# Ulixes-8/UNet-Implementations

Hardware: NVIDIA B200
Metric: our_unet_512_train_images_per_sec (higher is better)
Workload: dtype bf16

## Files before the change

### unet-implementations_b200/csrc/conv_common.cuh

```cuda
#pragma once
#include "common.cuh"

namespace b200 {

#ifdef B200UNET_INSTRUMENT
constexpr bool kInstr = true;
#else
constexpr bool kInstr = false;
#endif
constexpr int kProducerWarps = 4;
constexpr int kMmaWarp = 4;
constexpr int kEpiWarp0 = 5;
constexpr int kConvThreads = 32 * (kEpiWarp0 + 4);

static inline int make_act_map(CUtensorMap* m, const __nv_bfloat16* base, int64_t pitch, int N, int H, int W, int C,
                        int hstep, int wstep, int hoff, int woff, int boxC, int boxW, int boxH) {
  const int Hs = (H - hoff + hstep - 1) / hstep;
  const int Ws = (W - woff + wstep - 1) / wstep;
  if (Hs <= 0 || Ws <= 0) return set_error(kErrInvalid, "empty sub-lattice");
  uint64_t dims[4] = {(uint64_t)C, (uint64_t)Ws, (uint64_t)Hs, (uint64_t)N};
  uint64_t strides[3] = {(uint64_t)(wstep * pitch * 2), (uint64_t)(hstep * (int64_t)W * pitch * 2),
                         (uint64_t)((int64_t)H * W * pitch * 2)};
  uint32_t box[4] = {(uint32_t)boxC, (uint32_t)boxW, (uint32_t)boxH, 1};
  const CUtensorMapSwizzle swz = (boxC * 2 == 128) ? CU_TENSOR_MAP_SWIZZLE_128B
                                 : (boxC * 2 == 64) ? CU_TENSOR_MAP_SWIZZLE_64B
                                                    : CU_TENSOR_MAP_SWIZZLE_NONE;
  if (swz == CU_TENSOR_MAP_SWIZZLE_NONE) return set_error(kErrInvalid, "box channel count %d unsupported", boxC);
  return make_tmap_bf16(m, base + ((int64_t)hoff * W + woff) * pitch, 4, dims, strides, box, swz);
}

static inline int make_weight_map(CUtensorMap* m, const void* w, int rows, int K, int boxK, int boxRows) {
  uint64_t dims[2] = {(uint64_t)K, (uint64_t)rows};
  uint64_t strides[1] = {(uint64_t)K * 2};
  uint32_t box[2] = {(uint32_t)boxK, (uint32_t)boxRows};
  return make_tmap_bf16(m, w, 2, dims, strides, box,
                        boxK == 64 ? CU_TENSOR_MAP_SWIZZLE_128B : CU_TENSOR_MAP_SWIZZLE_64B);
}

static inline int pick_bn(int n_total) {
  if (n_total % 256 == 0) return 256;
  if (n_total % 128 == 0) return 128;
  if (n_total % 64 == 0) return 64;
  if (n_total % 32 == 0) return 32;
  return 0;
}
static inline int pick_bn_gconv(int n_total, int bk) {
  if (n_total == 96 && bk == 32) return 96;
  if ((n_total == 192 || n_total == 384) && bk == 64) return 192;
  return pick_bn(n_total);
}
static inline int pick_bk(int c) { return c % 64 == 0 ? 64 : (c % 32 == 0 ? 32 : 0); }


int launch_wgrad_finalize(const float* partial, float* dw, int S, int cin, int cout, cudaStream_t st);

struct BwdSums {
  const __nv_bfloat16* y;
  int64_t y_pitch;
  const float* a;
  const float* b;
  float slope;
};

bool nconv_supported(int k_channels, int n_channels, int stride, int W);
int nconv_stat_slots(int N, int H, int W);
int nconv_launch(const void* src, int64_t src_pitch, const void* wpack, void* out, int64_t out_pitch, float* stats, int N,
                 int H, int W, int k_channels, int n_channels, int rev, int stat_slots, cudaStream_t st,
                 const BwdSums* bs = nullptr);
bool pconv_supported(int k_channels, int n_channels, int stride, int W, int64_t src_pitch, int64_t out_pitch);
int pconv_stat_slots(int N, int H, int W);
int pconv_launch(const void* src, const void* wpack, void* out, float* stats, int N, int H, int W, int rev, int stat_slots,
                 cudaStream_t st, const BwdSums* bs = nullptr);
int conv_stat_slots(int N, int OH, int OW, int Cout);

bool wgradn_supported(int Cin, int Cout, int stride);
int64_t wgradn_workspace_bytes(int N, int H, int W, int Cin, int Cout);
int wgradn_launch(const b200unet_conv_wgrad_args* a, cudaStream_t st);

}
```

### unet-implementations_b200/csrc/conv_fprop_dgrad.cu

```cuda
#include "common.cuh"
#include "ptx.cuh"
#include "conv_common.cuh"
#include <stdlib.h>

namespace b200 {

constexpr int kTH = 16, kTW = 8;
constexpr int kMaxLoads = 4;
constexpr int kMaxTaps = 9;

struct ALoad {
  int dh, dw;
  int rows, cols;
  int ntaps;
  uint32_t a_hi;
  uint32_t mt_step16;
  uint32_t winoff16[kMaxTaps];
  int koff[kMaxTaps];
};

struct GConvParams {
  int N, OH, OW, tiles_w, tiles_h;
  int nloads, ntaps_total;
  int s1;
// ... 691 lines not shown
  GC(32, 256, 4, 4, false)
  GC(32, 128, 8, 4, false)
  GC(32, 96, 8, 4, false)
  GC(32, 96, 8, 1, true)
  GC(32, 64, 8, 4, false)
  GC(32, 64, 8, 1, true)
  GC(32, 32, 8, 4, false)
  GC(32, 32, 8, 1, true)
#undef GC
  return set_error(kErrUnsupported, "no gconv instantiation for BK=%d BN=%d", BK, BN);
}

}

using namespace b200;

extern "C" int b200unet_conv_fprop_partials(int N, int OH, int OW, int Cout) { return conv_stat_slots(N, OH, OW, Cout); }

extern "C" int b200unet_conv_fprop(const b200unet_conv_fprop_args* a, void* stream) {
  B200_CHECK_ARG(a && a->x && a->w && a->y, "conv_fprop: null pointer");
  B200_CHECK_ARG(a->stride == 1 || a->stride == 2, "conv_fprop: stride %d unsupported", a->stride);
  const int BK = pick_bk(a->Cin), BN = pick_bn_gconv(a->Cout, BK);
  if (!BK || !BN)
    return set_error(kErrUnsupported, "conv_fprop: Cin=%d Cout=%d outside the tensor-core envelope (multiples of 32)",
                     a->Cin, a->Cout);
  B200_CHECK_ARG(a->x_pitch % 8 == 0 && a->y_pitch % 8 == 0, "conv_fprop: pitches must be multiples of 8 elements");
  if (nconv_supported(a->Cin, a->Cout, a->stride, a->W))
    return nconv_launch(a->x, a->x_pitch, a->w, a->y, a->y_pitch, a->stats, a->N, a->H, a->W, a->Cin, a->Cout, 0,
                        conv_stat_slots(a->N, a->H, a->W, a->Cout), static_cast<cudaStream_t>(stream));
  const int s = a->stride;
  const int OH = (a->H - 1) / s + 1, OW = (a->W - 1) / s + 1;
  GConvParams p{};
  GConvMaps maps;
  p.N = a->N;
  p.OH = OH;
  p.OW = OW;
  p.mt = pick_mt(BK, BN, a->Cout, a->Cin, 9);
  p.tiles_w = ceil_div(OW, kTW);
  p.tiles_h = ceil_div(OH, kTH * p.mt);
  p.cin = a->Cin;
  p.cout = a->Cout;
  p.stats = a->stats;
  const __nv_bfloat16* x = static_cast<const __nv_bfloat16*>(a->x);
  TapSpec taps[9];
  SrcLattice lat[4];
  int rc;
  if (s == 1) {
    lat[0] = SrcLattice{x, a->x_pitch, a->N, a->H, a->W, a->Cin, 1, 1, 0, 0};
    int n = 0;
    for (int kw = 0; kw < 3; ++kw)
      for (int kh = 0; kh < 3; ++kh) taps[n++] = TapSpec{0, kh - 1, kw - 1, (kh * 3 + kw) * a->Cin};
  } else {
    B200_CHECK_ARG(a->H >= 2 && a->W >= 2, "conv_fprop: stride-2 input must be at least 2x2");
    for (int hp = 0; hp < 2; ++hp)
      for (int wp = 0; wp < 2; ++wp)
        lat[hp * 2 + wp] = SrcLattice{x, a->x_pitch, a->N, a->H, a->W, a->Cin, 2, 2, hp, wp};
    const int par[3] = {1, 0, 1}, sh[3] = {-1, 0, 0};
    int n = 0;
    for (int kw = 0; kw < 3; ++kw)
      for (int kh = 0; kh < 3; ++kh)
        taps[n++] = TapSpec{par[kh] * 2 + par[kw], sh[kh], sh[kw], (kh * 3 + kw) * a->Cin};
  }
  if ((rc = build_loads(taps, 9, lat, BK, &p, &maps))) return rc;
  const WSpec ws{a->w, a->Cout, 9 * a->Cin};
  const int OC = (BN % 64 == 0) ? 64 : 32;
  if ((rc = make_act_map(&maps.out[0], static_cast<const __nv_bfloat16*>(a->y), a->y_pitch, a->N, OH, OW, a->Cout, 1, 1, 0,
                         0, OC, kTW, kTH)))
    return rc;
  return dispatch_gconv(maps, p, ws, BK, BN, static_cast<cudaStream_t>(stream));
}

extern "C" int b200unet_conv_dgrad_bwd_slots(int N, int H, int W, int Cin, int Cout, int stride) {
  if (N <= 0 || H <= 0 || W <= 0) return 0;
  return nconv_supported(Cout, Cin, stride, W) ? nconv_stat_slots(N, H, W) : 0;
}

extern "C" int b200unet_conv_dgrad(const b200unet_conv_dgrad_args* a, void* stream) {
  B200_CHECK_ARG(a && a->dy && a->wt && a->dx, "conv_dgrad: null pointer");
  B200_CHECK_ARG(a->stride == 1 || a->stride == 2, "conv_dgrad: stride %d unsupported", a->stride);
  const int BK = pick_bk(a->Cout), BN = pick_bn_gconv(a->Cin, BK);
  if (!BK || !BN)
    return set_error(kErrUnsupported, "conv_dgrad: Cin=%d Cout=%d outside the tensor-core envelope", a->Cin, a->Cout);
  B200_CHECK_ARG(a->dx_pitch % 8 == 0 && a->dy_pitch % 8 == 0, "conv_dgrad: pitches must be multiples of 8 elements");
  if (nconv_supported(a->Cout, a->Cin, a->stride, a->W) && !a->dx2) {
    if (a->bs_part) {
      B200_CHECK_ARG(a->bs_y && a->bs_a && a->bs_b, "conv_dgrad: norm-backward sums need y, a and b");
      BwdSums bs{static_cast<const __nv_bfloat16*>(a->bs_y), a->bs_y_pitch, a->bs_a, a->bs_b, a->bs_slope};
      return nconv_launch(a->dy, a->dy_pitch, a->wt, a->dx, a->dx_pitch, a->bs_part, a->N, a->H, a->W, a->Cout, a->Cin, 1,
                          nconv_stat_slots(a->N, a->H, a->W), static_cast<cudaStream_t>(stream), &bs);
    }
    return nconv_launch(a->dy, a->dy_pitch, a->wt, a->dx, a->dx_pitch, nullptr, a->N, a->H, a->W, a->Cout, a->Cin, 1, 0,
                        static_cast<cudaStream_t>(stream));
  }
  B200_CHECK_ARG(!a->bs_part, "conv_dgrad: this shape does not produce norm-backward sums (b200unet_conv_dgrad_bwd_slots == 0)");
  const int s = a->stride;
  const int OH = (a->H - 1) / s + 1, OW = (a->W - 1) / s + 1;
  const __nv_bfloat16* dy = static_cast<const __nv_bfloat16*>(a->dy);
  const __nv_bfloat16* dx = static_cast<const __nv_bfloat16*>(a->dx);
  const int OC = (BN % 64 == 0) ? 64 : 32;
  cudaStream_t st = static_cast<cudaStream_t>(stream);
  int rc;
  GConvMaps maps;
  const WSpec ws{a->wt, a->Cin, 9 * a->Cout};
  SrcLattice lat[1] = {SrcLattice{dy, a->dy_pitch, a->N, OH, OW, a->Cout, 1, 1, 0, 0}};
  if (s == 1) {
    GConvParams p{};
    p.N = a->N;
    p.OH = a->H;
    p.OW = a->W;
    p.mt = pick_mt(BK, BN, a->Cin, a->Cout, 9);
    p.tiles_w = ceil_div(a->W, kTW);
    p.tiles_h = ceil_div(a->H, kTH * p.mt);
    p.cin = a->Cout;
    p.cout = a->Cin;
    p.stats = nullptr;
    TapSpec taps[9];
    int n = 0;
    for (int kw = 0; kw < 3; ++kw)
      for (int kh = 2; kh >= 0; --kh) taps[n++] = TapSpec{0, 1 - kh, 1 - kw, (kh * 3 + kw) * a->Cout};
    if ((rc = build_loads(taps, 9, lat, BK, &p, &maps))) return rc;
    if (a->dx2) {
      B200_CHECK_ARG(a->dx_split > 0 && a->dx_split < a->Cin && a->dx_split % OC == 0 && a->Cin / OC <= 8 && BN == a->Cin,
                     "conv_dgrad: dx_split=%d must be a multiple of %d inside (0, %d), one N tile", a->dx_split, OC, a->Cin);
      B200_CHECK_ARG(a->dx2_pitch % 8 == 0, "conv_dgrad: dx2 pitch must be a multiple of 8 elements");
      p.out_split = OC;
      const __nv_bfloat16* dx2 = static_cast<const __nv_bfloat16*>(a->dx2);
      for (int j = 0; j < a->Cin / OC; ++j) {
        const int c0 = j * OC;
        const bool first = c0 < a->dx_split;
        if ((rc = make_act_map(&maps.out[j], first ? dx + c0 : dx2 + (c0 - a->dx_split), first ? a->dx_pitch : a->dx2_pitch,
                               a->N, a->H, a->W, OC, 1, 1, 0, 0, OC, kTW, kTH)))
          return rc;
      }
      return dispatch_gconv(maps, p, ws, BK, BN, st);
    }
    if ((rc = make_act_map(&maps.out[0], dx, a->dx_pitch, a->N, a->H, a->W, a->Cin, 1, 1, 0, 0, OC, kTW, kTH))) return rc;
    return dispatch_gconv(maps, p, ws, BK, BN, st);
  }
  B200_CHECK_ARG(!a->dx2, "conv_dgrad: a split output needs stride 1");
  for (int ph = 0; ph < 2; ++ph)
    for (int pw = 0; pw < 2; ++pw) {
      const int Hs = (a->H - ph + 1) / 2, Ws = (a->W - pw + 1) / 2;
      if (Hs <= 0 || Ws <= 0) continue;
      GConvParams p{};
      p.N = a->N;
      p.OH = Hs;
      p.OW = Ws;
      p.mt = pick_mt(BK, BN, a->Cin, a->Cout, (ph ? 2 : 1) * (pw ? 2 : 1));
      p.tiles_w = ceil_div(Ws, kTW);
      p.tiles_h = ceil_div(Hs, kTH * p.mt);
      p.cin = a->Cout;
      p.cout = a->Cin;
      p.stats = nullptr;
      int khs[2], dhs[2], nkh, kws[2], dws[2], nkw;
      if (ph == 0) { nkh = 1; khs[0] = 1; dhs[0] = 0; } else { nkh = 2; khs[0] = 0; dhs[0] = 1; khs[1] = 2; dhs[1] = 0; }
      if (pw == 0) { nkw = 1; kws[0] = 1; dws[0] = 0; } else { nkw = 2; kws[0] = 0; dws[0] = 1; kws[1] = 2; dws[1] = 0; }
      TapSpec taps[4];
      int n = 0;
      for (int j = 0; j < nkw; ++j)
        for (int i = 0; i < nkh; ++i) taps[n++] = TapSpec{0, dhs[i], dws[j], (khs[i] * 3 + kws[j]) * a->Cout};
      if ((rc = build_loads(taps, n, lat, BK, &p, &maps))) return rc;
      if ((rc = make_act_map(&maps.out[0], dx, a->dx_pitch, a->N, a->H, a->W, a->Cin, 2, 2, ph, pw, OC, kTW, kTH)))
        return rc;
      if ((rc = dispatch_gconv(maps, p, ws, BK, BN, st))) return rc;
    }
  return 0;
// ... 71 lines not shown
```

### unet-implementations_b200/csrc/conv_narrow.cu

```cuda
#include "common.cuh"
#include "ptx.cuh"
#include "conv_common.cuh"
#include <stdlib.h>

namespace b200 {

constexpr int kNcTH = 4, kNcTW = 32, kNcValidW = 30;
constexpr int kNcPatchRows = kNcTH + 2;
constexpr int kNcProducers = 2, kNcMmaWarp = 2, kNcEpiWarp0 = 4;
constexpr int kNcMaxGroups = 3;

struct NConvParams {
  int N, H, W, tiles_w, tiles_h;
  int cin;
    int tiles_per_cta;
  int stat_slots;
  float* stats;
  long long* debug;
  BwdSums bs;
};

struct NConvMaps {
  CUtensorMap src;
  CUtensorMap w;
// ... 342 lines not shown
    tmem_dealloc(tmem_base, Cfg::kTmemCols);
  }
}

struct NConvGrid {
  int grid, tiles_per_cta, stat_slots, tiles_w, tiles_h;
};

static NConvGrid nconv_grid(int N, int H, int W) {
  NConvGrid g;
  g.tiles_w = ceil_div(W, kNcValidW);
  g.tiles_h = ceil_div(H, kNcTH);
  const long long per_img = static_cast<long long>(g.tiles_w) * g.tiles_h;
  const long long total = per_img * N;
  g.tiles_per_cta = static_cast<int>(ceil_div64(total, num_sms()));
  if (g.tiles_per_cta < 1) g.tiles_per_cta = 1;
  g.grid = static_cast<int>(ceil_div64(total, g.tiles_per_cta));
  g.stat_slots = 4 * kNcMaxGroups * (static_cast<int>(ceil_div64(per_img, g.tiles_per_cta)) + 1);
  return g;
}

static int nconv_bk(int k_channels) { return k_channels > 32 ? 64 : 32; }

bool nconv_supported(int k_channels, int n_channels, int stride, int W) {
  if (stride != 1 || (n_channels != 32 && n_channels != 64) || k_channels % 32 != 0 || k_channels <= 0) return false;
  if (W < 64) return false;
  {
    const char* e = getenv("B200UNET_NO_NCONV");
    if (e && atoi(e) == n_channels) return false;
  }
  const int BK = nconv_bk(k_channels);
  return static_cast<long long>(ceil_div(k_channels, BK)) * 3 * (3 * n_channels * BK * 2) <= 80 * 1024;
}

int nconv_stat_slots(int N, int H, int W) {
  const int a = nconv_grid(N, H, W).stat_slots, b = pconv_stat_slots(N, H, W);
  return a > b ? a : b;
}

static long long* nconv_debug_buffer() {
  static long long* buf = nullptr;
  static int state = -1;
  if (state < 0) {
    const char* e = getenv("B200UNET_GCONV_DEBUG");
    state = (e && e[0] == '1') ? 1 : 0;
    if (state) cudaMalloc(&buf, 148 * 8 * sizeof(long long));
  }
  return state ? buf : nullptr;
}

template <int BK, int CO, int A_SLOTS, bool REV, int NG>
static int launch_nconv(const NConvMaps& maps, NConvParams& p, const NConvGrid& g, cudaStream_t st) {
  using Cfg = NConvCfg<BK, CO, A_SLOTS, NG>;
  auto kern = nconv_kernel<BK, CO, A_SLOTS, REV, NG>;
  static bool attr_set = false;
  if (!attr_set) {
    B200_CUDA(cudaFuncSetAttribute(kern, cudaFuncAttributeMaxDynamicSharedMemorySize, Cfg::kSmemBytes));
    attr_set = true;
  }
  if (p.stats)
    B200_CUDA(cudaMemsetAsync(p.stats, 0, static_cast<size_t>(p.N) * p.stat_slots * CO * 2 * sizeof(float), st));
  p.debug = nconv_debug_buffer();
  if (kInstr && p.debug) cudaMemsetAsync(p.debug, 0, 148 * 8 * sizeof(long long), st);
  launch_k(kern, dim3(g.grid), dim3(Cfg::kThreads), Cfg::kSmemBytes, st, maps, p);
  B200_LAUNCH_CHECK("nconv_kernel");
  if (kInstr && p.debug) {
    long long h[8];
    cudaStreamSynchronize(st);
    cudaMemcpy(h, p.debug, sizeof(h), cudaMemcpyDeviceToHost);
    const long long tiles = g.tiles_per_cta, gt = (tiles + NG - 1) / NG;
    fprintf(stderr,
            "nconv<%d,%d,%d,%d,%d> K %d tiles/CTA %lld | per tile: producer0 wait %lld issue %lld | mma total %lld "
            "wait_tmem_empty %lld wait_a_full %lld | epilogue group 0 per ITS tile: total %lld wait_tmem_full %lld store+bar %lld\n",
            BK, CO, A_SLOTS, (int)REV, NG, p.cin, tiles, h[0] / tiles, h[1] / tiles, h[4] / tiles, h[2] / tiles, h[3] / tiles,
            h[6] / gt, h[5] / gt, h[7] / gt);
  }
  return 0;
}

int nconv_launch(const void* src, int64_t src_pitch, const void* wpack, void* out, int64_t out_pitch, float* stats, int N,
                 int H, int W, int k_channels, int n_channels, int rev, int stat_slots, cudaStream_t st, const BwdSums* bs) {
  if (pconv_supported(k_channels, n_channels, 1, W, src_pitch, out_pitch) && (!bs || bs->y_pitch == n_channels))
    return pconv_launch(src, wpack, out, stats, N, H, W, rev, stat_slots, st, bs);
  const int BK = nconv_bk(k_channels);
  const NConvGrid g = nconv_grid(N, H, W);
  NConvParams p{};
  NConvMaps maps;
  p.N = N;
  p.H = H;
  p.W = W;
  p.tiles_w = g.tiles_w;
  p.tiles_h = g.tiles_h;
  p.cin = k_channels;
  p.tiles_per_cta = g.tiles_per_cta;
  p.stat_slots = stat_slots > g.stat_slots ? stat_slots : g.stat_slots;
  p.stats = stats;
  if (bs) {
    if (!rev || !stats || bs->y_pitch % 2 != 0)
      return set_error(kErrInvalid, "nconv: the norm-backward sums need the data gradient and a partial buffer");
    p.bs = *bs;
  }
  int rc;
  if ((rc = make_act_map(&maps.src, static_cast<const __nv_bfloat16*>(src), src_pitch, N, H, W, k_channels, 1, 1, 0, 0, BK,
                         kNcTW, kNcPatchRows)))
    return rc;
  if ((rc = make_act_map(&maps.out, static_cast<const __nv_bfloat16*>(out), out_pitch, N, H, W, n_channels, 1, 1, 0, 0,
                         n_channels, kNcValidW, kNcTH)))
    return rc;
  {
    const uint64_t kc = static_cast<uint64_t>(k_channels);
    uint64_t dims[4] = {kc, 3, 3, static_cast<uint64_t>(n_channels)};
    uint64_t strides[3] = {kc * 2, 3 * kc * 2, 9 * kc * 2};
    uint32_t box[4] = {static_cast<uint32_t>(BK), 3, 1, static_cast<uint32_t>(n_channels)};
    if ((rc = make_tmap_bf16(&maps.w, wpack, 4, dims, strides, box,
                             BK == 64 ? CU_TENSOR_MAP_SWIZZLE_128B : CU_TENSOR_MAP_SWIZZLE_64B)))
      return rc;
  }
#define NC(bk, co, as, ng) \
  if (BK == bk && n_channels == co) \
    return rev ? launch_nconv<bk, co, as, true, ng>(maps, p, g, st) : launch_nconv<bk, co, as, false, ng>(maps, p, g, st);
  NC(64, 64, 4, 2) NC(64, 32, 4, 2) NC(32, 64, 8, 2) NC(32, 32, 8, 2)
#undef NC
  return set_error(kErrUnsupported, "no nconv instantiation for BK=%d N=%d", BK, n_channels);
}

}
```

### unet-implementations_b200/csrc/conv_pair.cu

```cuda
#include "common.cuh"
#include "ptx.cuh"
#include "conv_common.cuh"
#include <stdlib.h>

namespace b200 {

constexpr int kPcTH = 4, kPcTW = 32, kPcValidW = 30;
constexpr int kPcPatchRows = kPcTH + 2;
constexpr int kPcProducers = 2, kPcMmaWarp = 2, kPcEpiWarp0 = 4;
constexpr int kPcNG = 2;
constexpr int kPcStatWarp0 = kPcEpiWarp0 + 4 * kPcNG;
constexpr int kPcC = 32;
constexpr int kPcSlots = 6;

struct PConvParams {
  int N, H, Wp, tiles_w, tiles_h;
  int tiles_per_cta;
  int stat_slots;
  float* stats;
  const __nv_bfloat16* w;
  BwdSums bs;
};

struct PConvMaps {
// ... 317 lines not shown
      th = th_n;
      tw = tw_n;
      n_img = img_n;
    };
    for (int it = 0; it < n_tiles; it += 2) {
      one_tile(it, ya, yb);
      if (it + 1 < n_tiles) one_tile(it + 1, yb, ya);
    }
    if (acc_img >= 0) flush(acc_img);
  }

  tc_fence_before();
  __syncthreads();
  if (warp == kPcMmaWarp) {
    tc_fence_after();
    tmem_dealloc(tmem_base, Cfg::kTmemCols);
  }
}

struct PConvGrid {
  int grid, tiles_per_cta, stat_slots, tiles_w, tiles_h;
};

static PConvGrid pconv_grid(int N, int H, int W) {
  PConvGrid g;
  g.tiles_w = ceil_div(W / 2, kPcValidW);
  g.tiles_h = ceil_div(H, kPcTH);
  const long long per_img = static_cast<long long>(g.tiles_w) * g.tiles_h;
  const long long total = per_img * N;
  g.tiles_per_cta = static_cast<int>(ceil_div64(total, num_sms()));
  if (g.tiles_per_cta < 1) g.tiles_per_cta = 1;
  g.grid = static_cast<int>(ceil_div64(total, g.tiles_per_cta));
  g.stat_slots = 4 * kPcNG * (static_cast<int>(ceil_div64(per_img, g.tiles_per_cta)) + 1);
  return g;
}

bool pconv_supported(int k_channels, int n_channels, int stride, int W, int64_t src_pitch, int64_t out_pitch) {
  static const bool off = [] { const char* e = getenv("B200UNET_NO_PCONV"); return e && e[0] == '1'; }();
  return !off && stride == 1 && k_channels == kPcC && n_channels == kPcC && W % 2 == 0 && W >= 128 &&
         src_pitch == kPcC && out_pitch == kPcC;
}

int pconv_stat_slots(int N, int H, int W) { return (W % 2 == 0 && W >= 128) ? pconv_grid(N, H, W).stat_slots : 0; }

int pconv_launch(const void* src, const void* wpack, void* out, float* stats, int N, int H, int W, int rev, int stat_slots,
                 cudaStream_t st, const BwdSums* bs) {
  const PConvGrid g = pconv_grid(N, H, W);
  PConvParams p{};
  PConvMaps maps;
  p.N = N;
  p.H = H;
  p.Wp = W / 2;
  p.tiles_w = g.tiles_w;
  p.tiles_h = g.tiles_h;
  p.tiles_per_cta = g.tiles_per_cta;
  p.stat_slots = stat_slots > g.stat_slots ? stat_slots : g.stat_slots;
  p.stats = stats;
  p.w = static_cast<const __nv_bfloat16*>(wpack);
  if (bs) {
    if (!rev || !stats || bs->y_pitch != kPcC)
      return set_error(kErrInvalid, "pconv: the norm-backward sums need the data gradient, a partial buffer and a dense y");
    p.bs = *bs;
  }
  int rc;
  if ((rc = make_act_map(&maps.src, static_cast<const __nv_bfloat16*>(src), 64, N, H, W / 2, 64, 1, 1, 0, 0, 64, kPcTW,
                         kPcPatchRows)))
    return rc;
  if ((rc = make_act_map(&maps.out, static_cast<const __nv_bfloat16*>(out), 64, N, H, W / 2, 64, 1, 1, 0, 0, 64, kPcValidW,
                         kPcTH)))
    return rc;
  auto kern = rev ? pconv_kernel<true> : pconv_kernel<false>;
  static bool attr_set[2] = {false, false};
  if (!attr_set[rev ? 1 : 0]) {
    B200_CUDA(cudaFuncSetAttribute(kern, cudaFuncAttributeMaxDynamicSharedMemorySize, PConvCfg::kSmemBytes));
    attr_set[rev ? 1 : 0] = true;
  }
  if (p.stats)
    B200_CUDA(cudaMemsetAsync(p.stats, 0, static_cast<size_t>(p.N) * p.stat_slots * kPcC * 2 * sizeof(float), st));
  launch_k(kern, dim3(g.grid), dim3(PConvCfg::kThreads), PConvCfg::kSmemBytes, st, maps, p);
  B200_LAUNCH_CHECK("pconv_kernel");
  return 0;
}

}
```

### unet-implementations_b200/csrc/ptx.cuh

```cuda
#pragma once
#include <cuda.h>
#include <cuda_runtime.h>
#include <cuda_bf16.h>
#include <stdint.h>

namespace b200 {

__device__ __forceinline__ uint32_t smem_u32(const void* p) {
  return static_cast<uint32_t>(__cvta_generic_to_shared(p));
}

__device__ __forceinline__ bool elect_one() {
  uint32_t pred;
  asm volatile(
      "{\n\t.reg .pred P;\n\t"
      "elect.sync _|P, 0xffffffff;\n\t"
      "selp.b32 %0, 1, 0, P;\n\t}"
      : "=r"(pred));
  return pred != 0;
}

__device__ __forceinline__ void pdl_launch_dependents() { asm volatile("griddepcontrol.launch_dependents;" ::: "memory"); }
__device__ __forceinline__ void pdl_wait() { asm volatile("griddepcontrol.wait;" ::: "memory"); }

// ... 79 lines not shown
__device__ __forceinline__ void tma_store_4d(const CUtensorMap* m, const void* src, int c0, int c1, int c2, int c3) {
  asm volatile("cp.async.bulk.tensor.4d.global.shared::cta.tile.bulk_group [%0, {%2, %3, %4, %5}], [%1];" ::"l"(m),
               "r"(smem_u32(src)), "r"(c0), "r"(c1), "r"(c2), "r"(c3)
               : "memory");
}
__device__ __forceinline__ void tma_store_commit() { asm volatile("cp.async.bulk.commit_group;" ::: "memory"); }
__device__ __forceinline__ void tma_store_wait_all() { asm volatile("cp.async.bulk.wait_group 0;" ::: "memory"); }
__device__ __forceinline__ void tma_store_wait_read_all() {
  asm volatile("cp.async.bulk.wait_group.read 0;" ::: "memory");
}
__device__ __forceinline__ void tma_store_wait_read_1() {
  asm volatile("cp.async.bulk.wait_group.read 1;" ::: "memory");
}
__device__ __forceinline__ void fence_proxy_async_smem() {
  asm volatile("fence.proxy.async.shared::cta;" ::: "memory");
}

__device__ __forceinline__ void tmem_alloc(uint32_t* dst_smem, uint32_t ncols) {
  asm volatile("tcgen05.alloc.cta_group::1.sync.aligned.shared::cta.b32 [%0], %1;" ::"r"(smem_u32(dst_smem)),
               "r"(ncols)
               : "memory");
}
__device__ __forceinline__ void tmem_relinquish() {
  asm volatile("tcgen05.relinquish_alloc_permit.cta_group::1.sync.aligned;" ::: "memory");
}
__device__ __forceinline__ void tmem_dealloc(uint32_t taddr, uint32_t ncols) {
  asm volatile("tcgen05.dealloc.cta_group::1.sync.aligned.b32 %0, %1;" ::"r"(taddr), "r"(ncols) : "memory");
}
__device__ __forceinline__ void tc_fence_before() {
  asm volatile("tcgen05.fence::before_thread_sync;" ::: "memory");
}
__device__ __forceinline__ void tc_fence_after() { asm volatile("tcgen05.fence::after_thread_sync;" ::: "memory"); }

__device__ __forceinline__ void umma_bf16(uint32_t tmem_d, uint64_t adesc, uint64_t bdesc, uint32_t idesc,
                                          uint32_t accumulate) {
  asm volatile(
      "{\n\t.reg .pred p;\n\t"
      "setp.ne.b32 p, %4, 0;\n\t"
      "tcgen05.mma.cta_group::1.kind::f16 [%0], %1, %2, %3, p;\n\t}" ::"r"(tmem_d),
      "l"(adesc), "l"(bdesc), "r"(idesc), "r"(accumulate)
      : "memory");
}
__device__ __forceinline__ uint32_t umma_desc_lo(uint32_t saddr, uint32_t lbo_bytes) {
  return ((saddr >> 4) & 0x3FFFu) | (((lbo_bytes >> 4) & 0x3FFFu) << 16);
}
__host__ __device__ constexpr uint32_t umma_desc_hi(uint32_t sbo_bytes, uint32_t layout) {
  return ((sbo_bytes >> 4) & 0x3FFFu) | (1u << 14) | ((layout & 7u) << 29);
}
__device__ __forceinline__ void umma_bf16_lean(uint32_t tmem_d, uint32_t a_lo, uint32_t a_hi, uint32_t b_lo,
                                               uint32_t b_hi, uint32_t idesc, uint32_t accumulate) {
  asm volatile(
      "{\n\t.reg .pred p;\n\t.reg .b64 da, db;\n\t"
      "setp.ne.b32 p, %6, 0;\n\t"
      "mov.b64 da, {%1, %2};\n\t"
      "mov.b64 db, {%3, %4};\n\t"
      "tcgen05.mma.cta_group::1.kind::f16 [%0], da, db, %5, p;\n\t}" ::"r"(tmem_d),
      "r"(a_lo), "r"(a_hi), "r"(b_lo), "r"(b_hi), "r"(idesc), "r"(accumulate)
      : "memory");
}
__device__ __forceinline__ void umma_commit(uint64_t* bar) {
  asm volatile("tcgen05.commit.cta_group::1.mbarrier::arrive::one.shared::cluster.b64 [%0];" ::"r"(smem_u32(bar))
               : "memory");
}
__device__ __forceinline__ void tmem_ld_32x32(uint32_t taddr, uint32_t (&v)[32]) {
  asm volatile(
      "tcgen05.ld.sync.aligned.32x32b.x32.b32 "
      "{%0, %1, %2, %3, %4, %5, %6, %7, %8, %9, %10, %11, %12, %13, %14, %15, "
      "%16, %17, %18, %19, %20, %21, %22, %23, %24, %25, %26, %27, %28, %29, %30, %31}, [%32];"
      : "=r"(v[0]), "=r"(v[1]), "=r"(v[2]), "=r"(v[3]), "=r"(v[4]), "=r"(v[5]), "=r"(v[6]), "=r"(v[7]), "=r"(v[8]),
        "=r"(v[9]), "=r"(v[10]), "=r"(v[11]), "=r"(v[12]), "=r"(v[13]), "=r"(v[14]), "=r"(v[15]), "=r"(v[16]),
        "=r"(v[17]), "=r"(v[18]), "=r"(v[19]), "=r"(v[20]), "=r"(v[21]), "=r"(v[22]), "=r"(v[23]), "=r"(v[24]),
        "=r"(v[25]), "=r"(v[26]), "=r"(v[27]), "=r"(v[28]), "=r"(v[29]), "=r"(v[30]), "=r"(v[31])
      : "r"(taddr)
      : "memory");
}
__device__ __forceinline__ void tmem_ld_32x16(uint32_t taddr, uint32_t (&v)[16]) {
  asm volatile(
      "tcgen05.ld.sync.aligned.32x32b.x16.b32 "
      "{%0, %1, %2, %3, %4, %5, %6, %7, %8, %9, %10, %11, %12, %13, %14, %15}, [%16];"
      : "=r"(v[0]), "=r"(v[1]), "=r"(v[2]), "=r"(v[3]), "=r"(v[4]), "=r"(v[5]), "=r"(v[6]), "=r"(v[7]), "=r"(v[8]),
        "=r"(v[9]), "=r"(v[10]), "=r"(v[11]), "=r"(v[12]), "=r"(v[13]), "=r"(v[14]), "=r"(v[15])
      : "r"(taddr)
      : "memory");
}
__device__ __forceinline__ void tmem_ld_wait() { asm volatile("tcgen05.wait::ld.sync.aligned;" ::: "memory"); }

__device__ __forceinline__ uint32_t mapa_u32(uint32_t saddr, uint32_t rank) {
  uint32_t ra;
  asm volatile("mapa.shared::cluster.u32 %0, %1, %2;" : "=r"(ra) : "r"(saddr), "r"(rank));
  return ra;
}
__device__ __forceinline__ uint32_t cluster_ctarank() {
  uint32_t r;
  asm volatile("mov.u32 %0, %%cluster_ctarank;" : "=r"(r));
  return r;
}
__device__ __forceinline__ void cluster_sync_all() {
  asm volatile("barrier.cluster.arrive.release.aligned;" ::: "memory");
  asm volatile("barrier.cluster.wait.acquire.aligned;" ::: "memory");
}
__device__ __forceinline__ void tma_load_2d_pair(void* dst, const CUtensorMap* m, uint32_t leader_bar, int c0, int c1) {
  asm volatile(
      "cp.async.bulk.tensor.2d.cta_group::2.shared::cluster.global.mbarrier::complete_tx::bytes [%0], [%1, {%3, %4}], [%2];"
      ::"r"(smem_u32(dst)), "l"(m), "r"(leader_bar), "r"(c0), "r"(c1)
      : "memory");
}
__device__ __forceinline__ void tma_load_4d_pair(void* dst, const CUtensorMap* m, uint32_t leader_bar, int c0, int c1,
                                                 int c2, int c3) {
  asm volatile(
      "cp.async.bulk.tensor.4d.cta_group::2.shared::cluster.global.mbarrier::complete_tx::bytes [%0], [%1, {%3, %4, %5, "
      "%6}], [%2];" ::"r"(smem_u32(dst)),
      "l"(m), "r"(leader_bar), "r"(c0), "r"(c1), "r"(c2), "r"(c3)
      : "memory");
}
__device__ __forceinline__ void mbar_arrive_cluster(uint64_t* bar, uint32_t rank) {
  asm volatile(
      "{\n\t.reg .b32 ra;\n\t"
      "mapa.shared::cluster.u32 ra, %0, %1;\n\t"
      "mbarrier.arrive.release.cluster.shared::cluster.b64 _, [ra];\n\t}" ::"r"(smem_u32(bar)),
      "r"(rank)
      : "memory");
}
__device__ __forceinline__ void tmem_alloc_pair(uint32_t* dst_smem, uint32_t ncols) {
  asm volatile("tcgen05.alloc.cta_group::2.sync.aligned.shared::cta.b32 [%0], %1;" ::"r"(smem_u32(dst_smem)),
               "r"(ncols)
               : "memory");
}
__device__ __forceinline__ void tmem_relinquish_pair() {
  asm volatile("tcgen05.relinquish_alloc_permit.cta_group::2.sync.aligned;" ::: "memory");
}
__device__ __forceinline__ void tmem_dealloc_pair(uint32_t taddr, uint32_t ncols) {
  asm volatile("tcgen05.dealloc.cta_group::2.sync.aligned.b32 %0, %1;" ::"r"(taddr), "r"(ncols) : "memory");
}
__device__ __forceinline__ void umma_bf16_lean_pair(uint32_t tmem_d, uint32_t a_lo, uint32_t a_hi, uint32_t b_lo,
                                                    uint32_t b_hi, uint32_t idesc, uint32_t accumulate) {
  asm volatile(
      "{\n\t.reg .pred p;\n\t.reg .b64 da, db;\n\t"
      "setp.ne.b32 p, %6, 0;\n\t"
      "mov.b64 da, {%1, %2};\n\t"
      "mov.b64 db, {%3, %4};\n\t"
      "tcgen05.mma.cta_group::2.kind::f16 [%0], da, db, %5, p;\n\t}" ::"r"(tmem_d),
      "r"(a_lo), "r"(a_hi), "r"(b_lo), "r"(b_hi), "r"(idesc), "r"(accumulate)
      : "memory");
}
__device__ __forceinline__ void umma_commit_pair_u32(uint32_t bar) {
  asm volatile(
      "{\n\t.reg .b16 m;\n\t"
      "mov.b16 m, 3;\n\t"
      "tcgen05.commit.cta_group::2.mbarrier::arrive::one.shared::cluster.multicast::cluster.b64 [%0], m;\n\t}" ::"r"(bar)
      : "memory");
}

enum : uint32_t { kSwzNone = 0, kSwz128 = 2, kSwz64 = 4, kSwz32 = 6 };

__device__ __forceinline__ uint64_t umma_smem_desc(uint32_t saddr, uint32_t lbo_bytes, uint32_t sbo_bytes,
                                                   uint32_t layout) {
  uint64_t d = 0;
  d |= static_cast<uint64_t>((saddr >> 4) & 0x3FFF);
  d |= static_cast<uint64_t>((lbo_bytes >> 4) & 0x3FFF) << 16;
  d |= static_cast<uint64_t>((sbo_bytes >> 4) & 0x3FFF) << 32;
  d |= static_cast<uint64_t>(1) << 46;
  d |= static_cast<uint64_t>(layout & 7) << 61;
  return d;
}
__host__ __device__ constexpr uint32_t umma_idesc_bf16(int M, int N, int a_mn, int b_mn) {
  return (1u << 4) | (1u << 7) | (1u << 10) | (static_cast<uint32_t>(a_mn) << 15) |
// ... 44 lines not shown
```

Baseline: 1607.

## Add paired-column 96-channel conv kernel for fprop and dgrad

Adds a specialised tcgen05 kernel for 3x3 convolutions between 96 and 32 channels. It treats pairs of adjacent pixels as one wider pixel (W/2 lattice) so each MMA uses N=96 and the horizontal taps merge. Partial sums of neighbouring columns are combined with warp shuffles in the epilogue. Fprop fuses norm statistics in dedicated warps, and dgrad writes to split outputs through strided tensor maps. This replaces the narrow/generic paths for these shapes and adds complex swizzle and weight-repacking logic that must be correct.

```diff
diff --git a/unet-implementations_b200/csrc/conv_common.cuh b/unet-implementations_b200/csrc/conv_common.cuh
--- a/unet-implementations_b200/csrc/conv_common.cuh
+++ b/unet-implementations_b200/csrc/conv_common.cuh
@@ -71,6 +71,12 @@
 int pconv_stat_slots(int N, int H, int W);
 int pconv_launch(const void* src, const void* wpack, void* out, float* stats, int N, int H, int W, int rev, int stat_slots,
                  cudaStream_t st, const BwdSums* bs = nullptr);
+bool pconv96_fprop_supported(int k_channels, int n_channels, int stride, int W, int64_t src_pitch, int64_t out_pitch);
+int pconv96_fprop(const void* x, const void* wpack, void* y, float* stats, int N, int H, int W, int stat_slots,
+                  cudaStream_t st);
+bool pconv96_dgrad_supported(int cin, int cout, int stride, int W, int64_t dy_pitch);
+int pconv96_dgrad(const void* dy, const void* wpack, const void* const out[3], const int64_t pitch[3], int N, int H, int W,
+                  cudaStream_t st);
 int conv_stat_slots(int N, int OH, int OW, int Cout);
 
 bool wgradn_supported(int Cin, int Cout, int stride);
diff --git a/unet-implementations_b200/csrc/conv_fprop_dgrad.cu b/unet-implementations_b200/csrc/conv_fprop_dgrad.cu
--- a/unet-implementations_b200/csrc/conv_fprop_dgrad.cu
+++ b/unet-implementations_b200/csrc/conv_fprop_dgrad.cu
@@ -797,6 +797,25 @@
   if (!BK || !BN)
     return set_error(kErrUnsupported, "conv_dgrad: Cin=%d Cout=%d outside the tensor-core envelope", a->Cin, a->Cout);
   B200_CHECK_ARG(a->dx_pitch % 8 == 0 && a->dy_pitch % 8 == 0, "conv_dgrad: pitches must be multiples of 8 elements");
+  if (pconv96_dgrad_supported(a->Cin, a->Cout, a->stride, a->W, a->dy_pitch) && !a->bs_part) {
+    const __nv_bfloat16* dx = static_cast<const __nv_bfloat16*>(a->dx);
+    const void* out[3];
+    int64_t pitch[3];
+    for (int j = 0; j < 3; ++j) {
+      out[j] = dx + 32 * j;
+      pitch[j] = a->dx_pitch;
+    }
+    if (a->dx2) {
+      B200_CHECK_ARG(a->dx_split > 0 && a->dx_split < a->Cin && a->dx_split % 32 == 0,
+                     "conv_dgrad: dx_split=%d must be a multiple of 32 inside (0, %d)", a->dx_split, a->Cin);
+      B200_CHECK_ARG(a->dx2_pitch % 8 == 0, "conv_dgrad: dx2 pitch must be a multiple of 8 elements");
+      for (int j = a->dx_split / 32; j < 3; ++j) {
+        out[j] = static_cast<const __nv_bfloat16*>(a->dx2) + (32 * j - a->dx_split);
+        pitch[j] = a->dx2_pitch;
+      }
+    }
+    return pconv96_dgrad(a->dy, a->wt, out, pitch, a->N, a->H, a->W, static_cast<cudaStream_t>(stream));
+  }
   if (nconv_supported(a->Cout, a->Cin, a->stride, a->W) && !a->dx2) {
     if (a->bs_part) {
       B200_CHECK_ARG(a->bs_y && a->bs_a && a->bs_b, "conv_dgrad: norm-backward sums need y, a and b");
diff --git a/unet-implementations_b200/csrc/conv_narrow.cu b/unet-implementations_b200/csrc/conv_narrow.cu
--- a/unet-implementations_b200/csrc/conv_narrow.cu
+++ b/unet-implementations_b200/csrc/conv_narrow.cu
@@ -448,6 +448,8 @@
                  int H, int W, int k_channels, int n_channels, int rev, int stat_slots, cudaStream_t st, const BwdSums* bs) {
   if (pconv_supported(k_channels, n_channels, 1, W, src_pitch, out_pitch) && (!bs || bs->y_pitch == n_channels))
     return pconv_launch(src, wpack, out, stats, N, H, W, rev, stat_slots, st, bs);
+  if (!rev && pconv96_fprop_supported(k_channels, n_channels, 1, W, src_pitch, out_pitch))
+    return pconv96_fprop(src, wpack, out, stats, N, H, W, stat_slots, st);
   const int BK = nconv_bk(k_channels);
   const NConvGrid g = nconv_grid(N, H, W);
   NConvParams p{};
diff --git a/unet-implementations_b200/csrc/conv_pair.cu b/unet-implementations_b200/csrc/conv_pair.cu
--- a/unet-implementations_b200/csrc/conv_pair.cu
+++ b/unet-implementations_b200/csrc/conv_pair.cu
@@ -423,4 +423,435 @@
   return 0;
 }
 
-}
+constexpr int kP9K = 288;
+constexpr int kP9BTileBytes = 96 * 128;
+constexpr int kP9BTiles = kP9K / 64 + 1;
+
+template <bool REV>
+struct P9Cfg {
+  static constexpr int KC = REV ? 1 : 3;
+  static constexpr int OG = REV ? 3 : 1;
+  static constexpr int NG = REV ? 4 : 2;
+  static constexpr int kSlots = REV ? 4 : 5;
+  static constexpr int kStatWarp0 = kPcEpiWarp0 + 4 * NG;
+  static constexpr int kThreads = 32 * (kStatWarp0 + (REV ? 0 : 4));
+  static constexpr int kSlotBytes = kPcPatchRows * kPcTW * 128;
+  static constexpr int kBBytes = kP9BTiles * kP9BTileBytes;
+  static constexpr int kStageBufBytes = 16 * 1024;
+  static constexpr int kSmemBytes = kSlots * kSlotBytes + kBBytes + NG * kStageBufBytes + 1024;
+  static constexpr uint32_t kTmemCols = NG * 128;
+  static_assert(kSmemBytes <= 227 * 1024 - 256, "shared memory budget");
+};
+
+struct P9Params {
+  int N, H, Wp, tiles_w, tiles_h;
+  int tiles_per_cta;
+  int stat_slots;
+  float* stats;
+  const __nv_bfloat16* w;
+};
+
+struct P9Maps {
+  CUtensorMap src;
+  CUtensorMap out[6];
+};
+
+__device__ __forceinline__ void p9_mma(uint32_t d, uint32_t a_lo, uint32_t b_lo, bool par, bool first) {
+  constexpr uint32_t hi = umma_desc_hi(8 * 128, kSwz128);
+  constexpr uint32_t id32 = umma_idesc_bf16(128, 32, 0, 0), id64 = umma_idesc_bf16(128, 64, 0, 0),
+                     id96 = umma_idesc_bf16(128, 96, 0, 0);
+  constexpr uint32_t kRows32 = (32 * 128) >> 4, kRows64 = (64 * 128) >> 4;
+  if (!par) {
+    if (first) {
+      umma_bf16_lean(d, a_lo, hi, b_lo, hi, id32, 0u);
+      umma_bf16_lean(d + 32, a_lo, hi, b_lo + kRows32, hi, id64, 0u);
+    } else {
+      umma_bf16_lean(d, a_lo, hi, b_lo, hi, id96, 1u);
+    }
+  } else {
+    if (first) {
+      umma_bf16_lean(d + 32, a_lo, hi, b_lo, hi, id64, 1u);
+      umma_bf16_lean(d + 96, a_lo, hi, b_lo + kRows64, hi, id32, 0u);
+    } else {
+      umma_bf16_lean(d + 32, a_lo, hi, b_lo, hi, id96, 1u);
+    }
+  }
+}
+
+__device__ __forceinline__ constexpr uint32_t p9_b_off(int kk) {
+  return static_cast<uint32_t>((kk >> 6) * (kP9BTileBytes >> 4) + (((kk & 63) * 2) >> 4));
+}
+
+template <bool REV>
+__global__ void __launch_bounds__(P9Cfg<REV>::kThreads, 1) pconv96_kernel(const __grid_constant__ P9Maps maps,
+                                                                           const __grid_constant__ P9Params p) {
+  pdl_launch_dependents();
+  using Cfg = P9Cfg<REV>;
+  constexpr int KC = Cfg::KC, OG = Cfg::OG, NG = Cfg::NG, A_SLOTS = Cfg::kSlots;
+  extern __shared__ uint8_t smem_raw[];
+  __shared__ __align__(8) uint64_t a_full[A_SLOTS], a_empty[A_SLOTS];
+  __shared__ __align__(8) uint64_t b_full;
+  __shared__ __align__(8) uint64_t tmem_full_bar[NG], tmem_empty_bar[NG];
+  __shared__ uint32_t tmem_base_holder;
+
+  const int warp = threadIdx.x >> 5;
+  const int lane = threadIdx.x & 31;
+  uint8_t* smem = reinterpret_cast<uint8_t*>((reinterpret_cast<uintptr_t>(smem_raw) + 1023) & ~uintptr_t(1023));
+  uint8_t* smem_b = smem + A_SLOTS * Cfg::kSlotBytes;
+  uint8_t* staging = smem_b + Cfg::kBBytes;
+
+  const int tiles_per_img = p.tiles_w * p.tiles_h;
+  const int total_tiles = tiles_per_img * p.N;
+  const int tile_lo = min(static_cast<int>(blockIdx.x) * p.tiles_per_cta, total_tiles);
+  const int tile_hi = min(tile_lo + p.tiles_per_cta, total_tiles);
+
+  if (threadIdx.x == 0) {
+    for (int s = 0; s < A_SLOTS; ++s) {
+      mbar_init(&a_full[s], 1);
+      mbar_init(&a_empty[s], 1);
+    }
+    mbar_init(&b_full, NG * 128);
+    for (int b = 0; b < NG; ++b) {
+      mbar_init(&tmem_full_bar[b], 1);
+      mbar_init(&tmem_empty_bar[b], 4);
+    }
+    fence_barrier_init();
+  }
+  if (warp == kPcMmaWarp) {
+    tmem_alloc(&tmem_base_holder, Cfg::kTmemCols);
+    tmem_relinquish();
+  }
+  tc_fence_before();
+  __syncthreads();
+  tc_fence_after();
+  const uint32_t tmem_base = tmem_base_holder;
+  pdl_wait();
+
+  if (warp < kPcProducers) {
+    if (elect_one()) {
+      tma_prefetch_desc(&maps.src);
+      int b = 0;
+      for (int tile = tile_lo; tile < tile_hi; ++tile) {
+        const int n_img = tile / tiles_per_img;
+        const int t_in = tile - n_img * tiles_per_img;
+        const int tw_ = t_in / p.tiles_h;
+        const int h0 = (t_in - tw_ * p.tiles_h) * kPcTH, w0 = tw_ * kPcValidW;
+#pragma unroll
+        for (int c = 0; c < KC; ++c, ++b) {
+          if ((b % kPcProducers) != warp) continue;
+          const int slot = b % A_SLOTS;
+          const uint32_t ph = static_cast<uint32_t>((b / A_SLOTS) & 1);
+          mbar_wait(&a_empty[slot], ph ^ 1);
+          mbar_expect_tx(&a_full[slot], Cfg::kSlotBytes);
+          tma_load_4d(smem + slot * Cfg::kSlotBytes, &maps.src, &a_full[slot], 64 * c, w0 - 1, h0 - 1, n_img);
+        }
+      }
+    }
+  } else if (warp == kPcMmaWarp) {
+    if (elect_one()) {
+      constexpr uint32_t kSlot16 = Cfg::kSlotBytes >> 4, kWin16 = (kPcTW * 128) >> 4;
+      const uint32_t a_lo0 = umma_desc_lo(smem_u32(smem), 16);
+      const uint32_t b_lo0 = umma_desc_lo(smem_u32(smem_b), 16);
+      const uint32_t a_full0 = smem_u32(&a_full[0]), a_empty0 = smem_u32(&a_empty[0]);
+      mbar_wait(&b_full, 0);
+      tc_fence_after();
+      uint32_t aslot = 0, aph = 0;
+      int buf = 0;
+      uint32_t bph = 0;
+      for (int tile = tile_lo; tile < tile_hi; ++tile) {
+        if (!REV) {
+          mbar_wait(&tmem_empty_bar[buf], bph ^ 1);
+          tc_fence_after();
+          const uint32_t d = tmem_base + buf * 128;
+#pragma unroll
+          for (int c = 0; c < KC; ++c) {
+            mbar_wait_u32(a_full0 + aslot * 8, aph);
+            tc_fence_after();
+            const uint32_t a_lo = a_lo0 + aslot * kSlot16;
+#pragma unroll
+            for (int kh = 0; kh < 3; ++kh)
+#pragma unroll
+              for (int k = 0; k < 4; ++k) {
+                const int s = 4 * c + k;
+                const bool par = s >= 6;
+                p9_mma(d, a_lo + kh * kWin16 + 2 * k, b_lo0 + p9_b_off(kh * 96 + (par ? s - 6 : s) * 16), par,
+                       kh == 0 && (s == 0 || s == 6));
+              }
+            umma_commit_u32(a_empty0 + aslot * 8);
+            if (++aslot == A_SLOTS) { aslot = 0; aph ^= 1; }
+          }
+          umma_commit(&tmem_full_bar[buf]);
+          if (++buf == NG) { buf = 0; bph ^= 1; }
+        } else {
+          mbar_wait_u32(a_full0 + aslot * 8, aph);
+          tc_fence_after();
+          const uint32_t a_lo = a_lo0 + aslot * kSlot16;
+#pragma unroll
+          for (int g = 0; g < OG; ++g) {
+            mbar_wait(&tmem_empty_bar[buf], bph ^ 1);
+            tc_fence_after();
+            const uint32_t d = tmem_base + buf * 128;
+#pragma unroll
+            for (int kh = 0; kh < 3; ++kh)
+#pragma unroll
+              for (int k = 0; k < 4; ++k)
+                p9_mma(d, a_lo + kh * kWin16 + 2 * k, b_lo0 + p9_b_off((g * 3 + kh) * 32 + (k & 1) * 16), k >= 2,
+                       kh == 0 && (k & 1) == 0);
+            umma_commit(&tmem_full_bar[buf]);
+            if (++buf == NG) { buf = 0; bph ^= 1; }
+          }
+          umma_commit_u32(a_empty0 + aslot * 8);
+          if (++aslot == A_SLOTS) { aslot = 0; aph ^= 1; }
+        }
+      }
+    }
+  } else if (warp >= kPcEpiWarp0 && warp < Cfg::kStatWarp0) {
+    const int e = (warp - kPcEpiWarp0) >> 2;
+    const int q = warp & 3;
+    const int et = threadIdx.x - 32 * (kPcEpiWarp0 + 4 * e);
+    {
+      const int ft = threadIdx.x - 32 * kPcEpiWarp0;
+      for (int idx = ft; idx < kP9BTiles * 96 * 8; idx += NG * 128) {
+        const int t = idx / (96 * 8);
+        const int r = idx - t * (96 * 8);
+        const int n = r >> 3, c = r & 7;
+        const int kk = t * 64 + c * 8;
+        const int jb = n >> 5, co = n & 31;
+        uint4 v = make_uint4(0u, 0u, 0u, 0u);
+        if (kk < kP9K) {
+          if (!REV) {
+            const int kh = kk / 96, ci0 = kk - kh * 96;
+            v = __ldg(reinterpret_cast<const uint4*>(p.w + ((co * 3 + kh) * 3 + (2 - jb)) * 96 + ci0));
+          } else {
+            const int gk = kk >> 5, ci0 = kk & 31, g = gk / 3, kh = gk - 3 * g;
+            v = __ldg(reinterpret_cast<const uint4*>(p.w + (((32 * g + co) * 3 + (2 - kh)) * 3 + jb) * 32 + ci0));
+          }
+        }
+        *reinterpret_cast<uint4*>(smem_b + t * kP9BTileBytes + n * 128 + (((c ^ (n & 7)) & 7) << 4)) = v;
+      }
+      fence_proxy_async_smem();
+      mbar_arrive(&b_full);
+    }
+    const int bar_a = 1 + 2 * e, bar_b = 2 + 2 * e;
+    const bool do_stats = !REV && p.stats != nullptr;
+    const bool col_ok = lane >= 1 && lane <= kPcValidW;
+    const int srow = q * kPcValidW + lane - 1;
+    uint8_t* stg = staging + e * Cfg::kStageBufBytes;
+    const uint32_t t_addr = tmem_base + (static_cast<uint32_t>(q * 32) << 16) + e * 128;
+    const int n_units = (tile_hi - tile_lo) * OG;
+    uint32_t ph = 0;
+    for (int u = e; u < n_units; u += NG, ph ^= 1) {
+      const int it = u / OG, g = u - it * OG;
+      const int tile = tile_lo + it;
+      const int n_img = tile / tiles_per_img;
+      const int t_in = tile - n_img * tiles_per_img;
+      const int tw = t_in / p.tiles_h;
+      const int h0 = (t_in - tw * p.tiles_h) * kPcTH, w0 = tw * kPcValidW;
+      mbar_wait(&tmem_full_bar[e], ph);
+      tc_fence_after();
+      if (et == 0) tma_store_wait_read_all();
+      named_bar_sync(bar_a, 128);
+      if (do_stats && u != e) named_bar_sync(7 + e, 256);
+      const uint32_t base = smem_u32(stg) + srow * (REV ? 64 : 128);
+#pragma unroll 1
+      for (int o = 0; o < 4; ++o) {
+        uint32_t v3[8], v0[8], v1[8], v2[8];
+        tmem_ld_32x8(t_addr + 8 * o, v3);
+        tmem_ld_32x8(t_addr + 32 + 8 * o, v0);
+        tmem_ld_32x8(t_addr + 64 + 8 * o, v1);
+        tmem_ld_32x8(t_addr + 96 + 8 * o, v2);
+        tmem_ld_wait();
+        if (o == 3) {
+          tc_fence_before();
+          __syncwarp();
+          if (lane == 0) mbar_arrive(&tmem_empty_bar[e]);
+        }
+        float y0[8], y1[8];
+#pragma unroll
+        for (int c = 0; c < 8; ++c) {
+          y0[c] = __uint_as_float(v0[c]) + __shfl_up_sync(0xffffffffu, __uint_as_float(v2[c]), 1);
+          y1[c] = __uint_as_float(v1[c]) + __shfl_down_sync(0xffffffffu, __uint_as_float(v3[c]), 1);
+        }
+        if (col_ok) {
+          uint32_t a0, a1;
+          if (REV) {
+            a0 = base + (((o ^ (srow >> 1)) & 3) << 4);
+            a1 = a0 + 8192;
+          } else {
+            a0 = base + (((o ^ srow) & 7) << 4);
+            a1 = base + ((((4 + o) ^ srow) & 7) << 4);
+          }
+          asm volatile("st.shared.v4.b32 [%0], {%1, %2, %3, %4};" ::"r"(a0), "r"(pack_bf16x2(y0[0], y0[1])),
+                       "r"(pack_bf16x2(y0[2], y0[3])), "r"(pack_bf16x2(y0[4], y0[5])), "r"(pack_bf16x2(y0[6], y0[7]))
+                       : "memory");
+          asm volatile("st.shared.v4.b32 [%0], {%1, %2, %3, %4};" ::"r"(a1), "r"(pack_bf16x2(y1[0], y1[1])),
+                       "r"(pack_bf16x2(y1[2], y1[3])), "r"(pack_bf16x2(y1[4], y1[5])), "r"(pack_bf16x2(y1[6], y1[7]))
+                       : "memory");
+        }
+      }
+      fence_proxy_async_smem();
+      named_bar_sync(bar_b, 128);
+      if (et == 0) {
+        if (REV) {
+          tma_store_4d(&maps.out[2 * g], stg, 0, w0, h0, n_img);
+          tma_store_4d(&maps.out[2 * g + 1], stg + 8192, 0, w0, h0, n_img);
+        } else {
+          tma_store_4d(&maps.out[0], stg, 0, w0, h0, n_img);
+        }
+        tma_store_commit();
+      }
+      if (do_stats) named_bar_arrive(5 + e, 256);
+    }
+    if (et == 0) tma_store_wait_all();
+  } else if (!REV && warp >= Cfg::kStatWarp0 && p.stats != nullptr) {
+    const int q = warp & 3;
+    const int n_tiles = tile_hi - tile_lo;
+    float s1[8], s2[8];
+#pragma unroll
+    for (int i = 0; i < 8; ++i) s1[i] = s2[i] = 0.f;
+    int acc_img = -1;
+    auto flush = [&](int img) {
+      const int first_tile = img * tiles_per_img;
+      const int b0 = first_tile / p.tiles_per_cta;
+      const int slot = (static_cast<int>(blockIdx.x) - b0) * NG * 4 + q;
+      float* dst = p.stats + (static_cast<size_t>(img) * p.stat_slots + slot) * kPcC * 2;
+#pragma unroll
+      for (int i = 0; i < 8; ++i) {
+        float a = s1[i], b = s2[i];
+        a += __shfl_xor_sync(0xffffffffu, a, 8);
+        b += __shfl_xor_sync(0xffffffffu, b, 8);
+        a += __shfl_xor_sync(0xffffffffu, a, 16);
+        b += __shfl_xor_sync(0xffffffffu, b, 16);
+        a += __shfl_xor_sync(0xffffffffu, a, 4);
+        b += __shfl_xor_sync(0xffffffffu, b, 4);
+        s1[i] = a;
+        s2[i] = b;
+      }
+      if (lane < 4) {
+        float4* d4 = reinterpret_cast<float4*>(dst + 16 * lane);
+        d4[0] = make_float4(s1[0], s2[0], s1[1], s2[1]);
+        d4[1] = make_float4(s1[2], s2[2], s1[3], s2[3]);
+        d4[2] = make_float4(s1[4], s2[4], s1[5], s2[5]);
+        d4[3] = make_float4(s1[6], s2[6], s1[7], s2[7]);
+      }
+#pragma unroll
+      for (int i = 0; i < 8; ++i) s1[i] = s2[i] = 0.f;
+    };
+    const int rsub = lane >> 3, ch = lane & 7;
+    constexpr int kSteps = (kPcValidW + 3) / 4;
+    for (int it = 0; it < n_tiles; ++it) {
+      const int g = it % NG;
+      const uint8_t* stg = staging + g * Cfg::kStageBufBytes;
+      const int tile = tile_lo + it;
+      const int n_img = tile / tiles_per_img;
+      const int t_in = tile - n_img * tiles_per_img;
+      const int tw = t_in / p.tiles_h;
+      const int h0 = (t_in - tw * p.tiles_h) * kPcTH, w0 = tw * kPcValidW;
+      if (n_img != acc_img) {
+        if (acc_img >= 0) flush(acc_img);
+        acc_img = n_img;
+      }
+      const bool row_in = (h0 + q) < p.H;
+      named_bar_sync(5 + g, 256);
+#pragma unroll
+      for (int s = 0; s < kSteps; ++s) {
+        const int col = 4 * s + rsub;
+        const int r = q * kPcValidW + col;
+        uint4 w = make_uint4(0u, 0u, 0u, 0u);
+        if (row_in && col < kPcValidW && w0 + col < p.Wp)
+          w = lds_v4(smem_u32(stg) + r * 128 + (((ch ^ (r & 7)) & 7) << 4));
+        const uint32_t ww[4] = {w.x, w.y, w.z, w.w};
+#pragma unroll
+        for (int i = 0; i < 4; ++i) {
+          const float x0 = __uint_as_float(ww[i] << 16), x1 = __uint_as_float(ww[i] & 0xffff0000u);
+          s1[2 * i] += x0;
+          s2[2 * i] = fmaf(x0, x0, s2[2 * i]);
+          s1[2 * i + 1] += x1;
+          s2[2 * i + 1] = fmaf(x1, x1, s2[2 * i + 1]);
+        }
+      }
+      if (it + NG < n_tiles) named_bar_arrive(7 + g, 256);
+    }
+    if (acc_img >= 0) flush(acc_img);
+  }
+
+  tc_fence_before();
+  __syncthreads();
+  if (warp == kPcMmaWarp) {
+    tc_fence_after();
+    tmem_dealloc(tmem_base, Cfg::kTmemCols);
+  }
+}
+
+template <bool REV>
+static int launch_pconv96(const P9Maps& maps, const P9Params& p, const PConvGrid& g, cudaStream_t st) {
+  using Cfg = P9Cfg<REV>;
+  auto kern = pconv96_kernel<REV>;
+  static bool attr_set = false;
+  if (!attr_set) {
+    B200_CUDA(cudaFuncSetAttribute(kern, cudaFuncAttributeMaxDynamicSharedMemorySize, Cfg::kSmemBytes));
+    attr_set = true;
+  }
+  if (p.stats)
+    B200_CUDA(cudaMemsetAsync(p.stats, 0, static_cast<size_t>(p.N) * p.stat_slots * kPcC * 2 * sizeof(float), st));
+  launch_k(kern, dim3(g.grid), dim3(Cfg::kThreads), Cfg::kSmemBytes, st, maps, p);
+  B200_LAUNCH_CHECK("pconv96_kernel");
+  return 0;
+}
+
+static P9Params pconv96_params(const PConvGrid& g, const void* w, float* stats, int stat_slots, int N, int H, int W) {
+  P9Params p{};
+  p.N = N;
+  p.H = H;
+  p.Wp = W / 2;
+  p.tiles_w = g.tiles_w;
+  p.tiles_h = g.tiles_h;
+  p.tiles_per_cta = g.tiles_per_cta;
+  p.stat_slots = stat_slots > g.stat_slots ? stat_slots : g.stat_slots;
+  p.stats = stats;
+  p.w = static_cast<const __nv_bfloat16*>(w);
+  return p;
+}
+
+bool pconv96_fprop_supported(int k_channels, int n_channels, int stride, int W, int64_t src_pitch, int64_t out_pitch) {
+  return stride == 1 && k_channels == 96 && n_channels == kPcC && W % 2 == 0 && W >= 128 && src_pitch == 96 &&
+         out_pitch == kPcC;
+}
+
+int pconv96_fprop(const void* x, const void* wpack, void* y, float* stats, int N, int H, int W, int stat_slots,
+                  cudaStream_t st) {
+  const PConvGrid g = pconv_grid(N, H, W);
+  const P9Params p = pconv96_params(g, wpack, stats, stat_slots, N, H, W);
+  P9Maps maps;
+  int rc;
+  if ((rc = make_act_map(&maps.src, static_cast<const __nv_bfloat16*>(x), 192, N, H, W / 2, 192, 1, 1, 0, 0, 64, kPcTW,
+                         kPcPatchRows)))
+    return rc;
+  if ((rc = make_act_map(&maps.out[0], static_cast<const __nv_bfloat16*>(y), 64, N, H, W / 2, 64, 1, 1, 0, 0, 64,
+                         kPcValidW, kPcTH)))
+    return rc;
+  return launch_pconv96<false>(maps, p, g, st);
+}
+
+bool pconv96_dgrad_supported(int cin, int cout, int stride, int W, int64_t dy_pitch) {
+  return stride == 1 && cin == 96 && cout == kPcC && W % 2 == 0 && W >= 128 && dy_pitch == kPcC;
+}
+
+int pconv96_dgrad(const void* dy, const void* wpack, const void* const out[3], const int64_t pitch[3], int N, int H, int W,
+                  cudaStream_t st) {
+  const PConvGrid g = pconv_grid(N, H, W);
+  const P9Params p = pconv96_params(g, wpack, nullptr, 0, N, H, W);
+  P9Maps maps;
+  int rc;
+  if ((rc = make_act_map(&maps.src, static_cast<const __nv_bfloat16*>(dy), 64, N, H, W / 2, 64, 1, 1, 0, 0, 64, kPcTW,
+                         kPcPatchRows)))
+    return rc;
+  for (int j = 0; j < 3; ++j)
+    for (int par = 0; par < 2; ++par)
+      if ((rc = make_act_map(&maps.out[2 * j + par], static_cast<const __nv_bfloat16*>(out[j]), pitch[j], N, H, W, kPcC,
+                             1, 2, 0, par, kPcC, kPcValidW, kPcTH)))
+        return rc;
+  return launch_pconv96<true>(maps, p, g, st);
+}
+
+}
diff --git a/unet-implementations_b200/csrc/ptx.cuh b/unet-implementations_b200/csrc/ptx.cuh
--- a/unet-implementations_b200/csrc/ptx.cuh
+++ b/unet-implementations_b200/csrc/ptx.cuh
@@ -185,6 +185,12 @@
         "=r"(v[9]), "=r"(v[10]), "=r"(v[11]), "=r"(v[12]), "=r"(v[13]), "=r"(v[14]), "=r"(v[15])
       : "r"(taddr)
       : "memory");
+}
+__device__ __forceinline__ void tmem_ld_32x8(uint32_t taddr, uint32_t (&v)[8]) {
+  asm volatile("tcgen05.ld.sync.aligned.32x32b.x8.b32 {%0, %1, %2, %3, %4, %5, %6, %7}, [%8];"
+               : "=r"(v[0]), "=r"(v[1]), "=r"(v[2]), "=r"(v[3]), "=r"(v[4]), "=r"(v[5]), "=r"(v[6]), "=r"(v[7])
+               : "r"(taddr)
+               : "memory");
 }
 __device__ __forceinline__ void tmem_ld_wait() { asm volatile("tcgen05.wait::ld.sync.aligned;" ::: "memory"); }
 
```

Measured after the change: 1638 (median of 6 runs). 1.9% higher.
